# AjayGaneshC/medical-segmentation-pytorch

Measured on AMD Instinct MI355X. Metric: images/sec (whole node) + val Dice, DUCKNet-17 352x352 at 1/2/4/8 MI355X, higher is better.
Workload: dtype bf16; 1 GPU; model=DUCKNet-17, global_batch=320, per_gpu_batch=320, seq_len=123904, step=SegTrainer.train_step, image_size=352, parallelism=dp1, impl=fused, optimizer=adam, loss=ce, syncbn=False, hipgraph=True

## Files before the change

### csrc/bindings.cpp

```cpp
#include <torch/extension.h>
#include <c10/hip/HIPStream.h>

#include <algorithm>
#include <vector>

#include "launchers.h"

namespace {

hipStream_t cur_stream() { return c10::hip::getCurrentHIPStream().stream(); }

#define CHECK_DEV(t) TORCH_CHECK((t).is_cuda() && (t).is_contiguous(), #t " must be a contiguous GPU tensor")
#define CHECK_BF16(t) CHECK_DEV(t); TORCH_CHECK((t).scalar_type() == at::kBFloat16, #t " must be bf16")
#define CHECK_F32(t) CHECK_DEV(t); TORCH_CHECK((t).scalar_type() == at::kFloat, #t " must be fp32")
#define CHECK_I64(t) CHECK_DEV(t); TORCH_CHECK((t).scalar_type() == at::kLong, #t " must be int64")

inline uint16_t* bf(const at::Tensor& t) { return reinterpret_cast<uint16_t*>(t.data_ptr()); }
inline float* f32(const at::Tensor& t) { return t.data_ptr<float>(); }
inline const float* f32_opt(const c10::optional<at::Tensor>& t) {
  if (!t.has_value() || !t->defined()) return nullptr;
  CHECK_F32(*t);
  return t->data_ptr<float>();
}
inline float* f32_opt_mut(const c10::optional<at::Tensor>& t) { return const_cast<float*>(f32_opt(t)); }
// ... 1585 lines not shown
  a.Kp = (int)Kp_d;
  a.dxo = bf(dxo);
  if (bn_y.has_value() && bn_y->defined()) {
    CHECK_BF16(*bn_y); TORCH_CHECK(bn_y->numel() == nx, "bn_y numel");
    TORCH_CHECK(bn_coef.has_value() && stat_part.has_value(), "BN epilogue needs bn_coef and stat_part");
    CHECK_F32(*bn_coef); CHECK_F32(*stat_part);
    TORCH_CHECK(bn_coef->numel() >= 3 * g.Cgi && stat_part->numel() == nblk * 2 * g.Cgi, "BN epilogue shapes");
    a.bn_y = bf(*bn_y); a.bn_coef = bn_coef->data_ptr<float>(); a.stat_part = stat_part->data_ptr<float>();
  }
  a.bn_relu = bn_relu ? 1 : 0;
  a.dw = f32(dw);
  a.accum = accumulate ? 1 : 0;
  const int rc = conv_bwd_fused(a, g, cur_stream());
  TORCH_CHECK(rc == 0, "conv_bwd_fused: launch failed (", rc, ")");
}

}

extern "C" const char* msp_sources_sha();

PYBIND11_MODULE(_C, m) {
  m.doc() = "MI355X (gfx950) HIP kernels for medical_segmentation_pytorch_amd";
  m.def("conv_fwd", &conv_fwd, py::arg("xs"), py::arg("wp"), py::arg("ys"), py::arg("bias"), py::arg("stat_part"),
        py::arg("dims"), py::arg("dy"), py::arg("dx"), py::arg("trans"), py::arg("xc") = OptTensors{},
        py::arg("xrelu") = 0, py::arg("accumulate") = false, py::arg("gy") = OptTensors{},
        py::arg("gs") = OptTensors{}, py::arg("gk") = OptTensors{}, py::arg("grelu") = 0);
  m.def("conv_fwd_bn", &conv_fwd_bn, py::arg("xs"), py::arg("wp"), py::arg("ys"), py::arg("stat_part"), py::arg("dims"),
        py::arg("dy"), py::arg("dx"), py::arg("bn_y"), py::arg("bn_coef"), py::arg("relu"), py::arg("gy") = OptTensors{},
        py::arg("gs") = OptTensors{}, py::arg("gk") = OptTensors{}, py::arg("grelu") = 0);
  m.def("conv_wgrad", &conv_wgrad_t, py::arg("dys"), py::arg("xs"), py::arg("dw"), py::arg("dims"), py::arg("dy"),
        py::arg("dx"), py::arg("trans"), py::arg("xc") = OptTensors{}, py::arg("xrelu") = 0,
        py::arg("gy") = OptTensors{}, py::arg("gs") = OptTensors{}, py::arg("gk") = OptTensors{}, py::arg("grelu") = 0);
  m.def("conv_wgrad_uses_halo", &conv_wgrad_uses_halo_t);
  m.def("conv_pick_mi", &conv_pick_mi);
  m.def("conv_rows_alloc", &conv_rows_alloc);
  m.def("conv_stat_blocks", &conv_stat_blocks_t, py::arg("dims"), py::arg("dy"), py::arg("dx"), py::arg("trans") = false,
        py::arg("bwd") = false, py::arg("bne") = false);
  m.def("conv_uses_halo", &conv_uses_halo_t, py::arg("dims"), py::arg("dy"), py::arg("dx"), py::arg("trans"),
        py::arg("bwd") = false);
  m.def("conv_set_halo", [](bool on) { conv_set_halo(on ? 1 : 0); });
  m.def("conv_set_halo_split", [](int64_t mode) { conv_set_halo_split((int)mode); });
  m.def("conv_set_gemm", [](bool on) { conv_gemm_set(on ? 1 : 0); });
  m.def("conv_gemm_force_cfg", [](int64_t c) { conv_gemm_force_cfg((int)c); });
  m.def("conv_gemm_num_cfgs", []() { return conv_gemm_num_cfgs(); });
  m.def("conv_gemm_stamp_buffer", [](c10::optional<at::Tensor> buf) {
    if (!buf.has_value()) return conv_gemm_stamp_buffer(nullptr, 0);
    TORCH_CHECK(buf->is_cuda() && buf->is_contiguous() && buf->scalar_type() == at::kLong && buf->dim() == 2 &&
                    buf->size(1) == 4, "conv_gemm_stamp_buffer: a contiguous int64 [blocks][4] device tensor");
    return conv_gemm_stamp_buffer(buf->data_ptr(), buf->size(0));
  });
  m.def("conv_set_wgrad_gemm", [](int64_t mode) { conv_wgrad_gemm_set((int)mode); });
  m.def("conv_wgrad_gemm_force_cfg", [](int64_t c) { conv_wgrad_gemm_force_cfg((int)c); });
  m.def("conv_wgrad_gemm_num_cfgs", []() { return conv_wgrad_gemm_num_cfgs(); });
  m.def("conv_uses_wgrad_gemm", [](std::vector<int64_t> dims, std::vector<int64_t> dy, std::vector<int64_t> dx, bool trans) {
    return conv_wgrad_gemm_ok(make_geom(dims, dy, dx), trans);
  });
  m.def("conv_uses_gemm", [](std::vector<int64_t> dims, std::vector<int64_t> dy, std::vector<int64_t> dx, bool trans) {
    return conv_gemm_ok(make_geom(dims, dy, dx), trans);
  });
  m.def("conv_set_phase", [](bool on) { conv_set_phase(on ? 1 : 0); });
  m.def("pack_weight", &pack_weight_t);
  m.def("unpack_wgrad", &unpack_wgrad_t, py::arg("src"), py::arg("dst"), py::arg("nrow"), py::arg("nch"),
        py::arg("T"), py::arg("Cpk"), py::arg("Ktot"), py::arg("t_base"), py::arg("c_base"), py::arg("s_row"),
        py::arg("s_ch"), py::arg("accumulate"), py::arg("nrep") = 1, py::arg("rep_stride") = 0);
  m.def("conv_wgrad_replicas", &conv_wgrad_replicas_t, py::arg("dims"), py::arg("dy"), py::arg("dx"), py::arg("trans"),
        py::arg("bwd") = false, py::arg("pro") = false);
  m.def("pack_batch", &pack_batch_t);
  m.def("pack_per_block", &pack_per_block);
  m.def("bn_partial_blocks", [](int64_t P, int64_t Cp) { return bn_partial_blocks(P, Cp); });
  m.def("sum_stats", &sum_stats_t, py::arg("inputs"), py::arg("out"), py::arg("part"), py::arg("P"), py::arg("Cp"),
        py::arg("coefs") = OptTensors{}, py::arg("relu_mask") = 0);
  m.def("bn_reduce_partials", &bn_reduce_partials_t);
  m.def("bn_reduce_splits", [](int64_t nblk) { return bn_reduce_splits(nblk); });
  m.def("bn_collapse", &bn_collapse_t);
  m.def("bn_finalize", &bn_finalize_t);
  m.def("bn_reduce_finalize", &bn_reduce_finalize_t);
  m.def("bn_reduce_bwd_finalize", &bn_reduce_bwd_finalize_t);
  m.def("bn_rf_chunks", [](int64_t Cp) { return bn_rf_chunks((int)Cp); });
  m.def("bn_act_apply", &bn_act_apply_t);
  m.def("bn_act_apply_relu6", &bn_act_apply_relu6_t);
  m.def("bn_add_act", &bn_add_act_t);
  m.def("gconv_fwd", &gconv_fwd_t);
  m.def("relu6", &relu6_t);
  m.def("relu6_bwd", &relu6_bwd_t);
  m.def("bn_aug_mask", &bn_aug_mask_t);
  m.def("gconv_dgrad", &gconv_dgrad_t);
  m.def("gconv_wgrad_slices", &gconv_wgrad_slices_t);
  m.def("gconv_wgrad", &gconv_wgrad_t);
  m.def("gconv_mfma", &gconv_mfma_t);
  m.def("gconv_wgrad_mfma", &gconv_wgrad_mfma_t);
  m.def("gconv_wgrad_mfma_slices", &gconv_wgrad_mfma_slices_t);
  m.def("aug_gray_scratch_doubles", &aug_gray_scratch_doubles);
  m.def("bn_act_bwd_partial", &bn_act_bwd_partial_t);
  m.def("bn_bwd_finalize", &bn_bwd_finalize_t, py::arg("tmp"), py::arg("C"), py::arg("Cp"), py::arg("count"),
        py::arg("stats"), py::arg("dgamma"), py::arg("dbeta"), py::arg("coef"), py::arg("pscale") = 1.0);
  m.def("bn_act_bwd_apply", &bn_act_bwd_apply_t);
  m.def("bn_act_bwd_apply_part", &bn_act_bwd_apply_part_t);
  m.def("bn_tail_partial", &bn_tail_partial_t);
  m.def("bn_tail_apply", &bn_tail_apply_t, py::arg("dz"), py::arg("ys"), py::arg("ostats"), py::arg("ocoef"),
        py::arg("orelu"), py::arg("y"), py::arg("st"), py::arg("coef"), py::arg("relu_mask"), py::arg("dy"),
        py::arg("P"), py::arg("Cp"), py::arg("g") = py::none());
  m.def("bn_tail_blocks", [](int64_t P, int64_t Cp) { return bn_tail_blocks(P, (int)Cp); });
  m.attr("kTailMax") = kTailMax;
  m.attr("kTailMaxCp") = kTailMaxCp;
  m.def("nchw_to_nhwc", &nchw_to_nhwc_t);
  m.def("nhwc_to_nchw", &nhwc_to_nchw_t);
// ... 135 lines not shown
```

### csrc/conv_wgrad_gemm.hip

```cpp
#include <algorithm>

#include "common.h"
#include "launchers.h"

namespace {

typedef float f32x16_t __attribute__((ext_vector_type(16)));
typedef short s16x4_t __attribute__((ext_vector_type(4)));
typedef __attribute__((address_space(3))) uint8_t lds_u8_t;

DEVI f32x16_t mfma32(const uint4& a, const uint4& b, f32x16_t c) {
#ifdef GK_KO_MFMA
  c[0] += __uint_as_float(a.x ^ b.y);
  return c;
#else
  return __builtin_amdgcn_mfma_f32_32x32x16_bf16(as_bf16x8(a), as_bf16x8(b), c, 0, 0, 0);
#endif
}

__device__ __attribute__((aligned(64))) uint4 g_wg_zero_page[4];

DEVI void glds16(const void* src, uint32_t lds) {
#ifdef GK_KO_DMA
  return;
#endif
  unsigned keep;
  asm volatile("s_mov_b32 %0, m0\n\ts_mov_b32 m0, %2\n\ts_nop 0\n\tglobal_load_lds_dwordx4 %1, off\n\ts_mov_b32 m0, %0"
               : "=&s"(keep) : "v"(src), "s"(lds) : "memory");
}

DEVI uint2 tr_read(const uint8_t* p) {
#ifdef GK_KO_LDS
  return make_uint2((uint32_t)(uintptr_t)p, 1u);
#endif
  s16x4_t v = __builtin_amdgcn_ds_read_tr16_b64_v4i16((s16x4_t __attribute__((address_space(3)))*)(p));
  union { s16x4_t s; uint2 u; } c; c.s = v; return c.u;
}

struct FastDiv { uint32_t mul, shr; };
DEVI uint32_t fdiv_u(uint32_t n, FastDiv f) {
  return (uint32_t)(((uint64_t)__umulhi(n, f.mul) + n) >> f.shr);
}
FastDiv make_fastdiv(uint32_t d) {
  FastDiv f{0, 0};
  if (d <= 1) return f;
  uint32_t l = 0;
  while ((1ull << l) < d) ++l;
  f.mul = (uint32_t)((((1ull << l) - d) << 32) / d + 1);
  f.shr = l;
  return f;
}

constexpr int kBP = 64;

template <int R>
DEVI int chunk_swz(int row) { return R == 64 ? 0 : (R == 128 ? ((row >> 1) & 1) : (row & 3)); }

struct WgGeom {
  long M;
  int KT, n_co, n_k, stages_per_split, nstages;
  FastDiv d_ohw, d_ow;
  int kw, ty0, tys, tx0, txs;
};

template <int WM, int WN, int FM, int FN, bool PRO>
__global__ __launch_bounds__(64 * WM * WN, 2) void conv_wgrad_gemm_kernel(WgradPtrs P, float* __restrict__ dw,
                                                                          ConvGeom g, WgGeom wg) {
  constexpr int NW = WM * WN, NT = 64 * NW;
  constexpr int TCO = 32 * WM * FM, TK = 32 * WN * FN;
  constexpr int RA = TCO * 2, RB = TK * 2;
  constexpr int A_BYTES = kBP * RA, B_BYTES = kBP * RB, STAGE = A_BYTES + B_BYTES;
  constexpr int A_RPI = 1024 / RA, B_RPI = 1024 / RB;
  constexpr int A_INS = kBP / A_RPI / NW, B_INS = kBP / B_RPI / NW;
  static_assert((RA == 64 || RA == 128 || RA % 256 == 0) && (RB == 64 || RB == 128 || RB % 256 == 0), "row bytes");
  static_assert(RA <= 1024 && RB <= 1024 && A_INS * A_RPI * NW == kBP && B_INS * B_RPI * NW == kBP, "DMA split");
  static_assert(!PRO || B_RPI % 4 == 0, "prologue: one channel vector per lane (B rows <= 256 B)");
  extern __shared__ __attribute__((aligned(16))) uint8_t smem[];

  const int tid = threadIdx.x, lane = tid & 63, wave = __builtin_amdgcn_readfirstlane(tid >> 6);
  const uint32_t sbase = (uint32_t)(uintptr_t)(lds_u8_t*)smem;

  const int nwg = gridDim.x, orig = blockIdx.x;
  const int xq = nwg / 8, xr = nwg % 8, xcd = orig % 8;
  const int wgid = (xcd < xr ? xcd * (xq + 1) : xr * (xq + 1) + (xcd - xr) * xq) + orig / 8;
  const int ntile = wg.n_co * wg.n_k;
  const int split = wgid / ntile, tile = wgid - split * ntile;
  const int co_t = tile % wg.n_co, k_t = tile / wg.n_co;
  const int co0 = co_t * TCO, k0 = k_t * TK;
  const int rows = g.Go * g.Cgo, Cip = g.Gi * g.Cgi;
  const int st0 = split * wg.stages_per_split;
  const int nst = max(0, min(wg.stages_per_split, wg.nstages - st0));
  const uint16_t* zero = reinterpret_cast<const uint16_t*>(g_wg_zero_page);

  const uint16_t* a_base[A_INS];
  int a_row[A_INS];
#pragma unroll
  for (int j = 0; j < A_INS; ++j) {
    const int row = (j * NW + wave) * A_RPI + (lane * 16) / RA;
    const int slot = ((lane * 16) % RA) / 16;
    const int col = 32 * ((slot >> 2) ^ chunk_swz<RA>(row)) + 8 * (slot & 3);
    const int co = co0 + col;
    a_row[j] = row;
    if (co < rows) {
      const int og = co / g.Cgo;
      a_base[j] = P.dy[og] + (co - og * g.Cgo);
    } else {
      a_base[j] = nullptr;
    }
  }
  const uint16_t* b_base[B_INS];
  int b_row[B_INS], b_dy[B_INS], b_dx[B_INS];
  int b_ci = 0, b_gi = 0;
#pragma unroll
  for (int j = 0; j < B_INS; ++j) {
    const int row = (j * NW + wave) * B_RPI + (lane * 16) / RB;
    const int slot = ((lane * 16) % RB) / 16;
    const int col = 32 * ((slot >> 2) ^ chunk_swz<RB>(row)) + 8 * (slot & 3);
    const int k = k0 + col;
    b_row[j] = row;
    if (k < wg.KT) {
      const int t = k / Cip, rem = k - (k / Cip) * Cip;
      const int gi = rem / g.Cgi, ci = rem - gi * g.Cgi;
      const int tr = t / wg.kw, tc = t - (t / wg.kw) * wg.kw;
      b_dy[j] = wg.ty0 + tr * wg.tys;
      b_dx[j] = wg.tx0 + tc * wg.txs;
      const uint16_t* xg = P.x[0];
#pragma unroll
      for (int q = 1; q < kMaxGroups; ++q) xg = gi == q ? P.x[q] : xg;
      b_base[j] = xg + ci;
      b_ci = ci; b_gi = gi;
    } else {
      b_base[j] = nullptr; b_dy[j] = 0; b_dx[j] = 0;
    }
  }
  float psc[8], psh[8];
  bool prelu = false, pro_on = false;
  if constexpr (PRO) {
    const float* cf = P.xc[0];
#pragma unroll
    for (int q = 1; q < kMaxGroups; ++q) cf = b_gi == q ? P.xc[q] : cf;
    pro_on = cf != nullptr && b_base[0] != nullptr;
    prelu = (P.xrelu >> b_gi) & 1u;
#pragma unroll
    for (int e = 0; e < 8; ++e) { psc[e] = 1.f; psh[e] = 0.f; }
    if (pro_on) { load8f(cf + b_ci, psc); load8f(cf + g.Cgi + b_ci, psh); }
  }

  auto stage = [&](int s, uint32_t sb) -> unsigned {
    const long mb = (long)(st0 + s) * kBP;
#pragma unroll
    for (int j = 0; j < A_INS; ++j) {
      const long m = mb + a_row[j];
      const void* src = (a_base[j] != nullptr && m < wg.M) ? (const void*)(a_base[j] + m * g.Cgo) : (const void*)zero;
      glds16(src, sb + (j * NW + wave) * 1024);
    }
    unsigned ok = 0;
#pragma unroll
    for (int j = 0; j < B_INS; ++j) {
      const long m = mb + b_row[j];
      const void* src = zero;
      if (b_base[j] != nullptr && m < wg.M) {
        const uint32_t mu = (uint32_t)m;
        const uint32_t n = fdiv_u(mu, wg.d_ohw);
        const uint32_t r = mu - n * (uint32_t)(g.OH * g.OW);
        const uint32_t oh = fdiv_u(r, wg.d_ow);
        const int ow = (int)(r - oh * (uint32_t)g.OW);
        const int ih = (int)oh * g.stride + b_dy[j], iw = ow * g.stride + b_dx[j];
        if ((unsigned)ih < (unsigned)g.IH && (unsigned)iw < (unsigned)g.IW) {
          src = b_base[j] + ((long)((int)n * g.IH + ih) * g.IW + iw) * g.Cgi;
          ok |= 1u << j;
        }
      }
      glds16(src, sb + A_BYTES + (j * NW + wave) * 1024);
    }
    return ok;
  };

  const int wm = wave / WN, wn = wave - (wave / WN) * WN;
  const int gq = lane >> 4, li = lane & 15, lq = li >> 2, lp = li & 3;
  auto tr_addr = [&](int R, int row, int col) -> int {
    const int sw = R == 64 ? 0 : (R == 128 ? ((row >> 1) & 1) : (row & 3));
    return row * R + (((col >> 5) ^ sw) << 6) + ((col & 31) << 1);
  };
  int a_off[FM][2], b_off[FN][2];
#pragma unroll
  for (int i = 0; i < FM; ++i)
#pragma unroll
    for (int hh = 0; hh < 2; ++hh)
      a_off[i][hh] = tr_addr(RA, 8 * (gq >> 1) + 4 * hh + lq, wm * FM * 32 + i * 32 + 16 * (gq & 1) + 4 * lp);
#pragma unroll
  for (int j = 0; j < FN; ++j)
#pragma unroll
    for (int hh = 0; hh < 2; ++hh)
      b_off[j][hh] = A_BYTES + tr_addr(RB, 8 * (gq >> 1) + 4 * hh + lq, wn * FN * 32 + j * 32 + 16 * (gq & 1) + 4 * lp);

  f32x16_t acc[FM][FN];
#pragma unroll
  for (int i = 0; i < FM; ++i)
#pragma unroll
    for (int j = 0; j < FN; ++j)
#pragma unroll
      for (int e = 0; e < 16; ++e) acc[i][j][e] = 0.f;

  unsigned ok_cur = 0, ok_nxt = 0;
  if (nst > 0) ok_cur = stage(0, sbase);
  for (int s = 0; s < nst; ++s) {
    asm volatile("s_waitcnt vmcnt(0)" ::: "memory");
    const uint32_t cur = (s & 1) * STAGE;
    if constexpr (PRO) {
      if (pro_on) {
#pragma unroll
        for (int j = 0; j < B_INS; ++j) {
          if (!((ok_cur >> j) & 1u)) continue;
          uint4* v = reinterpret_cast<uint4*>(smem + cur + A_BYTES + (j * NW + wave) * 1024 + lane * 16);
          *v = affine8(*v, psc, psh, prelu);
        }
      }
      asm volatile("s_waitcnt lgkmcnt(0)" ::: "memory");
    }
    __builtin_amdgcn_s_barrier();
    __builtin_amdgcn_sched_barrier(0);
    if (s + 1 < nst) ok_nxt = stage(s + 1, sbase + ((s + 1) & 1) * STAGE);
    const uint8_t* sp = smem + cur;
#pragma unroll
    for (int ks = 0; ks < kBP / 16; ++ks) {
      uint4 af[FM], bf[FN];
#pragma unroll
      for (int i = 0; i < FM; ++i) {
        const uint2 lo = tr_read(sp + a_off[i][0] + ks * 16 * RA);
        const uint2 hi = tr_read(sp + a_off[i][1] + ks * 16 * RA);
        af[i] = make_uint4(lo.x, lo.y, hi.x, hi.y);
      }
#pragma unroll
      for (int j = 0; j < FN; ++j) {
        const uint2 lo = tr_read(sp + b_off[j][0] + ks * 16 * RB);
        const uint2 hi = tr_read(sp + b_off[j][1] + ks * 16 * RB);
        bf[j] = make_uint4(lo.x, lo.y, hi.x, hi.y);
      }
#pragma unroll
      for (int i = 0; i < FM; ++i)
#pragma unroll
        for (int j = 0; j < FN; ++j) acc[i][j] = mfma32(af[i], bf[j], acc[i][j]);
    }
    ok_cur = ok_nxt;
  }

  float* slab = dw + (long)split * rows * wg.KT;
  const int kc = k0 + wn * FN * 32 + (lane & 31);
  const int lh = lane >> 5;
#pragma unroll
  for (int j = 0; j < FN; ++j) {
    const int k = kc + 32 * j;
    if (k >= wg.KT) continue;
#pragma unroll
    for (int i = 0; i < FM; ++i)
#pragma unroll
      for (int e = 0; e < 16; ++e) {
        const int co = co0 + wm * FM * 32 + i * 32 + 8 * (e >> 2) + 4 * lh + (e & 3);
        if (co < rows) slab[(long)co * wg.KT + k] = acc[i][j][e];
      }
  }
}

constexpr bool wg_pro_ok(int wn, int fn) { return 32 * wn * fn <= 128; }

struct WgCfg { int wm, wn, fm, fn; };
constexpr WgCfg kWgCfgs[] = {
    {2, 2, 2, 2},
    {1, 4, 1, 1},
    {2, 2, 1, 2},
    {2, 2, 2, 1},
    {1, 4, 2, 1},
    {2, 2, 4, 1},
    {2, 4, 4, 2},
    {2, 4, 2, 2},
    {4, 2, 2, 2},
};
constexpr int kNumWgCfgs = sizeof(kWgCfgs) / sizeof(kWgCfgs[0]);

int g_wg_mode = -1;
int g_wg_cfg = -1;
constexpr long g_wg_blocks = 512;
constexpr double g_wg_stage_cost = 96.0;

void wg_env() {
  if (g_wg_mode < 0) {
    const char* e = getenv("MSP_WGRAD_GEMM");
    g_wg_mode = e == nullptr ? 1 : (e[0] == '0' ? 0 : (e[0] == '2' ? 2 : 1));
  }
}

int wg_pick(int rows, int KT, bool pro) {
  if (g_wg_cfg >= 0 && (!pro || wg_pro_ok(kWgCfgs[g_wg_cfg].wn, kWgCfgs[g_wg_cfg].fn))) return g_wg_cfg;
  int best = 0;
  double best_cost = 1e30;
  for (int c = 0; c < kNumWgCfgs; ++c) {
    if (pro && !wg_pro_ok(kWgCfgs[c].wn, kWgCfgs[c].fn)) continue;
    const int tco = 32 * kWgCfgs[c].wm * kWgCfgs[c].fm, tk = 32 * kWgCfgs[c].wn * kWgCfgs[c].fn;
    const double nt = (double)cdiv(rows, tco) * cdiv(KT, tk);
    const double cost = nt * ((double)tco * tk + g_wg_stage_cost * (tco + tk));
    if (cost < best_cost) { best_cost = cost; best = c; }
  }
  return best;
}

bool wg_tap_grid(const ConvGeom& g, WgGeom& w) {
  for (int kw = 1; kw <= g.T; ++kw) {
    if (g.T % kw != 0) continue;
    const int kh = g.T / kw;
    w.kw = kw; w.ty0 = g.dy[0]; w.tx0 = g.dx[0];
    w.tys = kh > 1 ? g.dy[kw] - g.dy[0] : 0;
    w.txs = kw > 1 ? g.dx[1] - g.dx[0] : 0;
    bool ok = true;
    for (int t = 0; t < g.T && ok; ++t) ok = g.dy[t] == w.ty0 + (t / kw) * w.tys && g.dx[t] == w.tx0 + (t % kw) * w.txs;
    if (ok) return true;
  }
  return false;
}

struct WgPlan { int cfg; WgGeom w; long blocks; int nsplit; };

WgPlan wg_plan(const ConvGeom& g, bool pro) {
  WgPlan p{};
  p.cfg = wg_pick(g.Go * g.Cgo, g.T * g.Gi * g.Cgi, pro);
  const WgCfg& c = kWgCfgs[p.cfg];
  WgGeom& w = p.w;
  (void)wg_tap_grid(g, w);
  w.M = (long)g.N * g.OH * g.OW;
  w.KT = g.T * g.Gi * g.Cgi;
  w.n_co = cdiv(g.Go * g.Cgo, 32 * c.wm * c.fm);
  w.n_k = cdiv(w.KT, 32 * c.wn * c.fn);
  w.nstages = (int)((w.M + kBP - 1) / kBP);
  const long ntile = (long)w.n_co * w.n_k;
  const long target = c.wm * c.wn >= 8 ? g_wg_blocks / 2 : g_wg_blocks;
  long ns = std::max(1L, std::min((long)w.nstages, target / std::max(1L, ntile)));
  w.stages_per_split = (int)((w.nstages + ns - 1) / ns);
  ns = (w.nstages + w.stages_per_split - 1) / w.stages_per_split;
  p.nsplit = (int)ns;
  p.blocks = ns * ntile;
  w.d_ohw = make_fastdiv((uint32_t)(g.OH * g.OW));
  w.d_ow = make_fastdiv((uint32_t)g.OW);
  return p;
}

template <int WM, int WN, int FM, int FN>
int launch_wg(const WgradPtrs& P, float* dw, const ConvGeom& g, const WgPlan& p, bool pro, hipStream_t s) {
  constexpr int LDS = 2 * kBP * (32 * WM * FM + 32 * WN * FN) * 2;
  static bool attr[2] = {false, false};
  if (pro) {
    if constexpr (!wg_pro_ok(WN, FN)) {
      return 1;
    } else {
    if (!attr[1]) {
      (void)hipFuncSetAttribute(reinterpret_cast<const void*>(&conv_wgrad_gemm_kernel<WM, WN, FM, FN, true>),
                                hipFuncAttributeMaxDynamicSharedMemorySize, LDS);
      attr[1] = true;
    }
    hipLaunchKernelGGL((conv_wgrad_gemm_kernel<WM, WN, FM, FN, true>), dim3((unsigned)p.blocks), dim3(64 * WM * WN),
                       LDS, s, P, dw, g, p.w);
    return 0;
    }
  }
  if (!attr[0]) {
    (void)hipFuncSetAttribute(reinterpret_cast<const void*>(&conv_wgrad_gemm_kernel<WM, WN, FM, FN, false>),
                              hipFuncAttributeMaxDynamicSharedMemorySize, LDS);
    attr[0] = true;
  }
  hipLaunchKernelGGL((conv_wgrad_gemm_kernel<WM, WN, FM, FN, false>), dim3((unsigned)p.blocks), dim3(64 * WM * WN), LDS,
                     s, P, dw, g, p.w);
  return 0;
}


}

bool conv_wgrad_gemm_ok(const ConvGeom& g, bool trans) {
  wg_env();
  if (!g_wg_mode || trans || g.Cgi % 8 != 0 || g.Cgo % 8 != 0) return false;
  WgGeom w{};
  if (!wg_tap_grid(g, w)) return false;
  const long M = (long)g.N * g.OH * g.OW;
  return M < (1L << 31) - 2 * kBP;
}

int conv_wgrad_gemm_replicas(const ConvGeom& g, bool pro) {
  wg_env();
  return wg_plan(g, pro).nsplit;
}

void conv_wgrad_gemm_set(int mode) { wg_env(); g_wg_mode = mode < 0 ? 0 : (mode > 2 ? 2 : mode); }
int conv_wgrad_gemm_mode() { wg_env(); return g_wg_mode; }
void conv_wgrad_gemm_force_cfg(int cfg) { wg_env(); g_wg_cfg = (cfg >= 0 && cfg < kNumWgCfgs) ? cfg : -1; }
int conv_wgrad_gemm_num_cfgs() { return kNumWgCfgs; }

int conv_wgrad_gemm(const WgradPtrs& P, float* dw, const ConvGeom& g, bool prologue, hipStream_t s) {
  const WgPlan p = wg_plan(g, prologue);
  switch (p.cfg) {
    case 0: return launch_wg<2, 2, 2, 2>(P, dw, g, p, prologue, s);
    case 1: return launch_wg<1, 4, 1, 1>(P, dw, g, p, prologue, s);
    case 2: return launch_wg<2, 2, 1, 2>(P, dw, g, p, prologue, s);
    case 3: return launch_wg<2, 2, 2, 1>(P, dw, g, p, prologue, s);
    case 4: return launch_wg<1, 4, 2, 1>(P, dw, g, p, prologue, s);
    case 5: return launch_wg<2, 2, 4, 1>(P, dw, g, p, prologue, s);
    case 6: return launch_wg<2, 4, 4, 2>(P, dw, g, p, prologue, s);
    case 7: return launch_wg<2, 4, 2, 2>(P, dw, g, p, prologue, s);
    case 8: return launch_wg<4, 2, 2, 2>(P, dw, g, p, prologue, s);
  }
  return 1;
}
```

### csrc/launchers.h

```cpp
#pragma once
#include <hip/hip_runtime.h>
#include <stdint.h>

constexpr int kMaxTaps = 49;

constexpr int kMaxGroups = 8;
struct ConvGeom {
  int N, IH, IW;
  int Gi, Cgi;
  int OH, OW;
  int Go, Cgo, Cgo_l;
  int T, Kp;
  int stride;
  int dy[kMaxTaps], dx[kMaxTaps];
};

struct ConvArgs {
  const uint16_t* x[kMaxGroups];
  uint16_t* y[kMaxGroups];
  const uint16_t* w;
  const float* bias;
  float* stat_part;
  const uint16_t* bn_y;
  const float* bn_coef;
  int bn_relu;
  const float* xc[kMaxGroups];
  unsigned xrelu;
  int accum;
  const uint16_t* gy[kMaxGroups];
  const float* gs[kMaxGroups];
  const float* gk[kMaxGroups];
  unsigned grelu;
  ConvGeom g;
};

struct WgradPtrs {
  const uint16_t* dy[kMaxGroups];
  const uint16_t* x[kMaxGroups];
  const float* xc[kMaxGroups];
  unsigned xrelu;
  const uint16_t* gy[kMaxGroups];
  const float* gs[kMaxGroups];
  const float* gk[kMaxGroups];
  unsigned grelu;
};

bool conv_wgrad_gemm_ok(const ConvGeom& g, bool trans);
int conv_wgrad_gemm_replicas(const ConvGeom& g, bool pro = false);
int conv_wgrad_gemm(const WgradPtrs& P, float* dw, const ConvGeom& g, bool prologue, hipStream_t s);
void conv_wgrad_gemm_set(int mode);
int conv_wgrad_gemm_mode();
void conv_wgrad_gemm_force_cfg(int cfg);
int conv_wgrad_gemm_num_cfgs();

int conv_pick_mi(int rows);
int conv_rows_alloc(int rows);
void conv_set_halo(int on);
void conv_set_halo_split(int mode);
void conv_set_phase(int on);
bool conv_uses_halo(const ConvGeom& g, bool trans, bool bwd = false);
long conv_stat_blocks(const ConvGeom& g, bool trans = false, bool bwd = false, bool bne = false);
bool conv_wgrad_uses_halo(const ConvGeom& g, bool trans);
int conv_igemm(const ConvArgs& a, bool trans, hipStream_t s);
const char* conv_error_string(int rc);

bool conv_gemm_ok(const ConvGeom& g, bool trans);
long conv_gemm_stat_blocks(const ConvGeom& g);
int conv_gemm(const ConvArgs& a, hipStream_t s);
int conv_gemm_phase(const ConvArgs& a, const int* tA, int KW, int s_, int py, int px, int OHf, int OWf,
                    hipStream_t s);
void conv_gemm_set(int on);
void conv_gemm_force_cfg(int cfg);
int conv_gemm_num_cfgs();
int conv_gemm_stamp_buffer(void* buf, long cap);
int conv_plan_selfcheck(int verbose);
int conv_wgrad_replicas(const ConvGeom& g, bool trans, bool bwd = false, bool pro = false);
int conv_wgrad(const uint16_t* const* dy, const uint16_t* const* x, float* dw, const ConvGeom& g, bool trans,
               const float* const* xc, unsigned xrelu, hipStream_t s, const uint16_t* const* gy = nullptr,
               const float* const* gs = nullptr, const float* const* gk = nullptr, unsigned grelu = 0);
void pack_weight(const float* src, uint16_t* dst, int nrow, int nch, int T, int Cpk, int Kp, int t_base,
                 int c_base, long s_row, long s_ch, hipStream_t s);
void pack_batch(const int64_t* jobs, const int* prefix, int njobs, int total_blocks, hipStream_t s);
int pack_per_block();
void unpack_wgrad(const float* src, float* dst, int nrow, int nch, int T, int Cpk, int Ktot, int t_base, int c_base,
                  long s_row, long s_ch, bool accumulate, int nrep, long rep_stride, hipStream_t s);

constexpr int kMaxSumInputs = 8;
constexpr int kTailMax = 6;
constexpr int kTailMaxCp = 512;
long bn_partial_blocks(long P, int Cp);
long bn_tail_blocks(long P, int Cp);
void bn_tail_partial(const uint16_t* dz, const uint16_t* ys, const float* ostats, const float* ocoef, int orelu, int k,
                     const uint16_t* const* y, const float* const* st, unsigned relu, float* part, long P, int Cp,
                     hipStream_t s);
void bn_tail_apply(const uint16_t* dz, const uint16_t* ys, const float* ostats, const float* ocoef, int orelu, int k,
                   const uint16_t* const* y, const float* const* st, const float* const* coef, unsigned relu,
                   uint16_t* const* dy, long P, int Cp, hipStream_t s, uint16_t* g = nullptr);
void sum_stats(const uint16_t* const* inputs, const float* const* coefs, unsigned relu_mask, int k, uint16_t* out,
               float* part, long P, int Cp, hipStream_t s);
int bn_reduce_splits(long nblk);
void bn_reduce_partials(const float* part, long nblk, int width, int col_off, int Cp, double* tmp, hipStream_t s);
void bn_collapse(const double* tmp, int S, int Cp, double* out, hipStream_t s);
void bn_finalize(const double* tmp, int S, int C, int Cp, float count, const float* gamma, const float* beta,
                 float* running_mean, float* running_var, float momentum, float eps, int training,
                 float* scale, float* shift, float* mean, float* invstd, hipStream_t s);
int bn_rf_chunks(int Cp);
// ... 283 lines not shown
```

Before: 687.9 images/sec.

## Add multi-stage LDS ring pipeline and incremental addressing to wgrad GEMM

Turns the weight-gradient GEMM's fixed double buffer into a configurable NS-stage ring with a BP-pixel stage depth. Global-to-LDS DMA issues are interleaved across the k-slices of the MFMA loop, and vmcnt waits are partial instead of full drains. Per-stage pixel-to-(n,oh,ow) divisions are replaced by incremental carry-based pointer advances, and an m0 save/restore is dropped. The 96K-LDS configs now default to a 3-stage ring, which uses more LDS per block and may lower occupancy. Split-count override and timestamp instrumentation hooks are also added.

New measurement: 687.8 images/sec. No clear change (-0.0%).

```diff
diff --git a/csrc/bindings.cpp b/csrc/bindings.cpp
--- a/csrc/bindings.cpp
+++ b/csrc/bindings.cpp
@@ -1661,6 +1661,24 @@
   m.def("conv_set_wgrad_gemm", [](int64_t mode) { conv_wgrad_gemm_set((int)mode); });
   m.def("conv_wgrad_gemm_force_cfg", [](int64_t c) { conv_wgrad_gemm_force_cfg((int)c); });
   m.def("conv_wgrad_gemm_num_cfgs", []() { return conv_wgrad_gemm_num_cfgs(); });
+  m.def("conv_wgrad_gemm_force_splits", [](int64_t n) { conv_wgrad_gemm_force_splits((int)n); });
+  m.def("conv_wgrad_gemm_ring", [](int64_t c) {
+    int ns = 0, bp = 0;
+    bool pro = false;
+    TORCH_CHECK(conv_wgrad_gemm_ring((int)c, &ns, &bp, &pro), "conv_wgrad_gemm_ring: no configuration ", c);
+    return std::make_tuple(ns, bp, pro);
+  });
+  m.def("conv_wgrad_gemm_forced", []() {
+    int cfg = -1, ns = -1;
+    conv_wgrad_gemm_forced(&cfg, &ns);
+    return std::make_pair(cfg, ns);
+  });
+  m.def("conv_wgrad_gemm_stamp_buffer", [](c10::optional<at::Tensor> buf) {
+    if (!buf.has_value()) return conv_wgrad_gemm_stamp_buffer(nullptr, 0);
+    TORCH_CHECK(buf->is_cuda() && buf->is_contiguous() && buf->scalar_type() == at::kLong && buf->dim() == 2 &&
+                    buf->size(1) == 6, "conv_wgrad_gemm_stamp_buffer: a contiguous int64 [blocks][6] device tensor");
+    return conv_wgrad_gemm_stamp_buffer(buf->data_ptr(), buf->size(0));
+  });
   m.def("conv_uses_wgrad_gemm", [](std::vector<int64_t> dims, std::vector<int64_t> dy, std::vector<int64_t> dx, bool trans) {
     return conv_wgrad_gemm_ok(make_geom(dims, dy, dx), trans);
   });
diff --git a/csrc/conv_wgrad_gemm.hip b/csrc/conv_wgrad_gemm.hip
--- a/csrc/conv_wgrad_gemm.hip
+++ b/csrc/conv_wgrad_gemm.hip
@@ -1,4 +1,5 @@
 #include <algorithm>
+#include <type_traits>
 
 #include "common.h"
 #include "launchers.h"
@@ -20,13 +21,27 @@
 
 __device__ __attribute__((aligned(64))) uint4 g_wg_zero_page[4];
 
+#ifdef GK_STAMP
+DEVI unsigned long long wg_clock() {
+  unsigned long long t;
+  __builtin_amdgcn_sched_barrier(0);
+  asm volatile("s_memrealtime %0\n\ts_waitcnt lgkmcnt(0)" : "=s"(t)::"memory");
+  __builtin_amdgcn_sched_barrier(0);
+  return t;
+}
+#endif
+
 DEVI void glds16(const void* src, uint32_t lds) {
 #ifdef GK_KO_DMA
   return;
 #endif
-  unsigned keep;
-  asm volatile("s_mov_b32 %0, m0\n\ts_mov_b32 m0, %2\n\ts_nop 0\n\tglobal_load_lds_dwordx4 %1, off\n\ts_mov_b32 m0, %0"
-               : "=&s"(keep) : "v"(src), "s"(lds) : "memory");
+  asm volatile("s_mov_b32 m0, %1\n\ts_nop 0\n\tglobal_load_lds_dwordx4 %0, off" ::"v"(src), "s"(lds) : "memory");
+}
+
+template <int N>
+DEVI void wait_vm() {
+  static_assert(N >= 0 && N < 64, "vmcnt is a 6-bit count");
+  asm volatile("s_waitcnt vmcnt(%0)" ::"n"(N) : "memory");
 }
 
 DEVI uint2 tr_read(const uint8_t* p) {
@@ -51,7 +66,7 @@
   return f;
 }
 
-constexpr int kBP = 64;
+constexpr int kSplitPx = 64;
 
 template <int R>
 DEVI int chunk_swz(int row) { return R == 64 ? 0 : (R == 128 ? ((row >> 1) & 1) : (row & 3)); }
@@ -61,21 +76,35 @@
   int KT, n_co, n_k, stages_per_split, nstages;
   FastDiv d_ohw, d_ow;
   int kw, ty0, tys, tx0, txs;
+  int q_n, q_oh, q_ow;
+  long img_bytes, img_step0, img_step1;
+#ifdef GK_STAMP
+  unsigned long long* stamp;
+  long stamp_cap;
+#endif
 };
 
-template <int WM, int WN, int FM, int FN, bool PRO>
+template <int WM, int WN, int FM, int FN, bool PRO, int NS, int BP>
 __global__ __launch_bounds__(64 * WM * WN, 2) void conv_wgrad_gemm_kernel(WgradPtrs P, float* __restrict__ dw,
                                                                           ConvGeom g, WgGeom wg) {
   constexpr int NW = WM * WN, NT = 64 * NW;
   constexpr int TCO = 32 * WM * FM, TK = 32 * WN * FN;
   constexpr int RA = TCO * 2, RB = TK * 2;
-  constexpr int A_BYTES = kBP * RA, B_BYTES = kBP * RB, STAGE = A_BYTES + B_BYTES;
+  constexpr int A_BYTES = BP * RA, B_BYTES = BP * RB, STAGE = A_BYTES + B_BYTES;
   constexpr int A_RPI = 1024 / RA, B_RPI = 1024 / RB;
-  constexpr int A_INS = kBP / A_RPI / NW, B_INS = kBP / B_RPI / NW;
+  constexpr int A_INS = BP / A_RPI / NW, B_INS = BP / B_RPI / NW;
+  constexpr int NI = A_INS + B_INS;
+  constexpr int KS = BP / 16;
+  static_assert(NS >= 2 && NS <= 5 && BP % 16 == 0 && kSplitPx % BP == 0, "ring");
   static_assert((RA == 64 || RA == 128 || RA % 256 == 0) && (RB == 64 || RB == 128 || RB % 256 == 0), "row bytes");
-  static_assert(RA <= 1024 && RB <= 1024 && A_INS * A_RPI * NW == kBP && B_INS * B_RPI * NW == kBP, "DMA split");
+  static_assert(RA <= 1024 && RB <= 1024 && A_INS * A_RPI * NW == BP && B_INS * B_RPI * NW == BP, "DMA split");
   static_assert(!PRO || B_RPI % 4 == 0, "prologue: one channel vector per lane (B rows <= 256 B)");
+  static_assert((NS - 1) * B_INS <= 32, "in-image masks of the stages in flight: one 32-bit queue");
   extern __shared__ __attribute__((aligned(16))) uint8_t smem[];
+#ifdef GK_STAMP
+  const unsigned long long ts0 = wg_clock();
+  unsigned long long ts1 = ts0, tsb = 0, bsum = 0;
+#endif
 
   const int tid = threadIdx.x, lane = tid & 63, wave = __builtin_amdgcn_readfirstlane(tid >> 6);
   const uint32_t sbase = (uint32_t)(uintptr_t)(lds_u8_t*)smem;
@@ -88,11 +117,13 @@
   const int co_t = tile % wg.n_co, k_t = tile / wg.n_co;
   const int co0 = co_t * TCO, k0 = k_t * TK;
   const int rows = g.Go * g.Cgo, Cip = g.Gi * g.Cgi;
-  const int st0 = split * wg.stages_per_split;
-  const int nst = max(0, min(wg.stages_per_split, wg.nstages - st0));
-  const uint16_t* zero = reinterpret_cast<const uint16_t*>(g_wg_zero_page);
-
-  const uint16_t* a_base[A_INS];
+  const long px0 = (long)split * wg.stages_per_split * kSplitPx;
+  const long px1 = min(wg.M, px0 + (long)wg.stages_per_split * kSplitPx);
+  const int nst = px1 > px0 ? (int)((px1 - px0 + BP - 1) / BP) : 0;
+  const uint8_t* zero = reinterpret_cast<const uint8_t*>(g_wg_zero_page);
+  asm volatile("" : "+s"(zero));
+
+  const uint8_t* a_ptr[A_INS];
   int a_row[A_INS];
 #pragma unroll
   for (int j = 0; j < A_INS; ++j) {
@@ -100,80 +131,87 @@
     const int slot = ((lane * 16) % RA) / 16;
     const int col = 32 * ((slot >> 2) ^ chunk_swz<RA>(row)) + 8 * (slot & 3);
     const int co = co0 + col;
-    a_row[j] = row;
     if (co < rows) {
       const int og = co / g.Cgo;
-      a_base[j] = P.dy[og] + (co - og * g.Cgo);
+      a_ptr[j] = reinterpret_cast<const uint8_t*>(P.dy[og] + (co - og * g.Cgo) + (px0 + row) * g.Cgo);
+      a_row[j] = row;
     } else {
-      a_base[j] = nullptr;
-    }
-  }
-  const uint16_t* b_base[B_INS];
-  int b_row[B_INS], b_dy[B_INS], b_dx[B_INS];
+      a_ptr[j] = zero;
+      a_row[j] = 1 << 30;
+    }
+  }
+  const int a_step = BP * g.Cgo * 2;
+  int rem = (int)min(wg.M - px0, (long)(1 << 29));
+  const uint8_t* b_img[B_INS];
+  int b_n[B_INS], b_oh[B_INS], b_ow[B_INS], b_dy[B_INS], b_dx[B_INS];
   int b_ci = 0, b_gi = 0;
+  bool b_k0 = false;
 #pragma unroll
   for (int j = 0; j < B_INS; ++j) {
     const int row = (j * NW + wave) * B_RPI + (lane * 16) / RB;
     const int slot = ((lane * 16) % RB) / 16;
     const int col = 32 * ((slot >> 2) ^ chunk_swz<RB>(row)) + 8 * (slot & 3);
     const int k = k0 + col;
-    b_row[j] = row;
+    const uint32_t mu = (uint32_t)(px0 + row);
+    const uint32_t n = fdiv_u(mu, wg.d_ohw);
+    const uint32_t r = mu - n * (uint32_t)(g.OH * g.OW);
+    const uint32_t oh = fdiv_u(r, wg.d_ow);
+    b_n[j] = (int)n; b_oh[j] = (int)oh; b_ow[j] = (int)(r - oh * (uint32_t)g.OW);
     if (k < wg.KT) {
-      const int t = k / Cip, rem = k - (k / Cip) * Cip;
-      const int gi = rem / g.Cgi, ci = rem - gi * g.Cgi;
+      const int t = k / Cip, rm = k - (k / Cip) * Cip;
+      const int gi = rm / g.Cgi, ci = rm - gi * g.Cgi;
       const int tr = t / wg.kw, tc = t - (t / wg.kw) * wg.kw;
       b_dy[j] = wg.ty0 + tr * wg.tys;
       b_dx[j] = wg.tx0 + tc * wg.txs;
       const uint16_t* xg = P.x[0];
 #pragma unroll
       for (int q = 1; q < kMaxGroups; ++q) xg = gi == q ? P.x[q] : xg;
-      b_base[j] = xg + ci;
+      b_img[j] = reinterpret_cast<const uint8_t*>(xg + ci) + (long)n * wg.img_bytes;
       b_ci = ci; b_gi = gi;
+      if (j == 0) b_k0 = true;
     } else {
-      b_base[j] = nullptr; b_dy[j] = 0; b_dx[j] = 0;
-    }
-  }
+      b_img[j] = zero; b_dy[j] = -(1 << 22); b_dx[j] = 0;
+    }
+  }
+  const int cgi2 = g.Cgi * 2;
   float psc[8], psh[8];
   bool prelu = false, pro_on = false;
   if constexpr (PRO) {
     const float* cf = P.xc[0];
 #pragma unroll
     for (int q = 1; q < kMaxGroups; ++q) cf = b_gi == q ? P.xc[q] : cf;
-    pro_on = cf != nullptr && b_base[0] != nullptr;
+    pro_on = cf != nullptr && b_k0;
     prelu = (P.xrelu >> b_gi) & 1u;
 #pragma unroll
     for (int e = 0; e < 8; ++e) { psc[e] = 1.f; psh[e] = 0.f; }
     if (pro_on) { load8f(cf + b_ci, psc); load8f(cf + g.Cgi + b_ci, psh); }
   }
 
-  auto stage = [&](int s, uint32_t sb) -> unsigned {
-    const long mb = (long)(st0 + s) * kBP;
-#pragma unroll
-    for (int j = 0; j < A_INS; ++j) {
-      const long m = mb + a_row[j];
-      const void* src = (a_base[j] != nullptr && m < wg.M) ? (const void*)(a_base[j] + m * g.Cgo) : (const void*)zero;
+  auto issue = [&](int i, uint32_t sb, unsigned& ok) {
+    if (i < A_INS) {
+      const int j = i;
+      const void* src = a_row[j] < rem ? (const void*)a_ptr[j] : (const void*)zero;
       glds16(src, sb + (j * NW + wave) * 1024);
-    }
-    unsigned ok = 0;
-#pragma unroll
-    for (int j = 0; j < B_INS; ++j) {
-      const long m = mb + b_row[j];
-      const void* src = zero;
-      if (b_base[j] != nullptr && m < wg.M) {
-        const uint32_t mu = (uint32_t)m;
-        const uint32_t n = fdiv_u(mu, wg.d_ohw);
-        const uint32_t r = mu - n * (uint32_t)(g.OH * g.OW);
-        const uint32_t oh = fdiv_u(r, wg.d_ow);
-        const int ow = (int)(r - oh * (uint32_t)g.OW);
-        const int ih = (int)oh * g.stride + b_dy[j], iw = ow * g.stride + b_dx[j];
-        if ((unsigned)ih < (unsigned)g.IH && (unsigned)iw < (unsigned)g.IW) {
-          src = b_base[j] + ((long)((int)n * g.IH + ih) * g.IW + iw) * g.Cgi;
-          ok |= 1u << j;
-        }
-      }
+      a_ptr[j] += a_step;
+    } else {
+      const int j = i - A_INS;
+      const int ih = __mul24(b_oh[j], g.stride) + b_dy[j], iw = __mul24(b_ow[j], g.stride) + b_dx[j];
+      const bool in = (b_n[j] < g.N) & ((unsigned)ih < (unsigned)g.IH) & ((unsigned)iw < (unsigned)g.IW);
+      const uint32_t off = __umul24(__umul24((unsigned)ih, (unsigned)g.IW) + (unsigned)iw, (unsigned)cgi2);
+      const uint8_t* at = b_img[j] + off;
+      asm volatile("" : "+v"(at));
+      const void* src = in ? (const void*)at : (const void*)zero;
       glds16(src, sb + A_BYTES + (j * NW + wave) * 1024);
-    }
-    return ok;
+      ok |= in ? (1u << j) : 0u;
+      int ow = b_ow[j] + wg.q_ow;
+      const bool c1 = ow >= g.OW;
+      b_ow[j] = c1 ? ow - g.OW : ow;
+      int oh = b_oh[j] + wg.q_oh + (c1 ? 1 : 0);
+      const bool c2 = oh >= g.OH;
+      b_oh[j] = c2 ? oh - g.OH : oh;
+      b_n[j] += wg.q_n + (c2 ? 1 : 0);
+      b_img[j] += c2 ? wg.img_step1 : wg.img_step0;
+    }
   };
 
   const int wm = wave / WN, wn = wave - (wave / WN) * WN;
@@ -202,28 +240,51 @@
 #pragma unroll
       for (int e = 0; e < 16; ++e) acc[i][j][e] = 0.f;
 
-  unsigned ok_cur = 0, ok_nxt = 0;
-  if (nst > 0) ok_cur = stage(0, sbase);
-  for (int s = 0; s < nst; ++s) {
-    asm volatile("s_waitcnt vmcnt(0)" ::: "memory");
-    const uint32_t cur = (s & 1) * STAGE;
+  int cb = 0, ib = 0;
+  unsigned okq = 0;
+#pragma unroll
+  for (int p = 0; p < NS - 1; ++p) {
+    if (p < nst) {
+      unsigned ok = 0;
+#pragma unroll
+      for (int i = 0; i < NI; ++i) issue(i, sbase + ib * STAGE, ok);
+      okq |= ok << (p * B_INS);
+      rem -= BP;
+      ++ib;
+    }
+  }
+  if (ib == NS) ib = 0;
+
+  auto iter = [&](auto infl, const bool more, const bool first) {
+    constexpr int INFL = decltype(infl)::value;
+    wait_vm<INFL * NI>();
+    const uint32_t cur = cb * STAGE;
     if constexpr (PRO) {
       if (pro_on) {
 #pragma unroll
         for (int j = 0; j < B_INS; ++j) {
-          if (!((ok_cur >> j) & 1u)) continue;
+          if (!((okq >> j) & 1u)) continue;
           uint4* v = reinterpret_cast<uint4*>(smem + cur + A_BYTES + (j * NW + wave) * 1024 + lane * 16);
           *v = affine8(*v, psc, psh, prelu);
         }
       }
-      asm volatile("s_waitcnt lgkmcnt(0)" ::: "memory");
-    }
+    }
+    asm volatile("s_waitcnt lgkmcnt(0)" ::: "memory");
     __builtin_amdgcn_s_barrier();
     __builtin_amdgcn_sched_barrier(0);
-    if (s + 1 < nst) ok_nxt = stage(s + 1, sbase + ((s + 1) & 1) * STAGE);
+#ifdef GK_STAMP
+    tsb = wg_clock();
+#endif
+    const uint32_t nxt = sbase + ib * STAGE;
+    unsigned ok = 0;
     const uint8_t* sp = smem + cur;
 #pragma unroll
-    for (int ks = 0; ks < kBP / 16; ++ks) {
+    for (int ks = 0; ks < KS; ++ks) {
+      if (more) {
+#pragma unroll
+        for (int i = 0; i < NI; ++i)
+          if ((i * KS) / NI == ks) issue(i, nxt, ok);
+      }
       uint4 af[FM], bf[FN];
 #pragma unroll
       for (int i = 0; i < FM; ++i) {
@@ -237,13 +298,41 @@
         const uint2 hi = tr_read(sp + b_off[j][1] + ks * 16 * RB);
         bf[j] = make_uint4(lo.x, lo.y, hi.x, hi.y);
       }
+#ifdef GK_STAMP
+      if (ks == 0) {
+        const unsigned long long t = wg_clock();
+        bsum += t - tsb;
+        if (first) ts1 = t;
+      }
+#endif
 #pragma unroll
       for (int i = 0; i < FM; ++i)
 #pragma unroll
         for (int j = 0; j < FN; ++j) acc[i][j] = mfma32(af[i], bf[j], acc[i][j]);
     }
-    ok_cur = ok_nxt;
-  }
+    okq >>= B_INS;
+    cb = cb + 1 == NS ? 0 : cb + 1;
+    if (more) {
+      okq |= ok << ((NS - 2) * B_INS);
+      rem -= BP;
+      ib = ib + 1 == NS ? 0 : ib + 1;
+    }
+  };
+
+  int s = 0;
+  for (; s + (NS - 2) < nst; ++s) iter(std::integral_constant<int, NS - 2>{}, s + NS - 1 < nst, s == 0);
+  if constexpr (NS >= 5) {
+    if (nst - 1 - s == 2) { iter(std::integral_constant<int, 2>{}, false, s == 0); ++s; }
+  }
+  if constexpr (NS >= 4) {
+    if (nst - 1 - s == 1) { iter(std::integral_constant<int, 1>{}, false, s == 0); ++s; }
+  }
+  if constexpr (NS >= 3) {
+    if (nst - 1 - s == 0) { iter(std::integral_constant<int, 0>{}, false, s == 0); ++s; }
+  }
+#ifdef GK_STAMP
+  const unsigned long long ts2 = wg_clock();
+#endif
 
   float* slab = dw + (long)split * rows * wg.KT;
   const int kc = k0 + wn * FN * 32 + (lane & 31);
@@ -260,26 +349,51 @@
         if (co < rows) slab[(long)co * wg.KT + k] = acc[i][j][e];
       }
   }
+#ifdef GK_STAMP
+  const unsigned long long ts3 = wg_clock();
+  if (tid == 0 && wg.stamp != nullptr && wgid < wg.stamp_cap) {
+    unsigned long long* sp = wg.stamp + 6 * (long)wgid;
+    sp[0] = ts0; sp[1] = ts1; sp[2] = ts2; sp[3] = ts3; sp[4] = bsum; sp[5] = (unsigned long long)nst;
+  }
+#endif
 }
 
 constexpr bool wg_pro_ok(int wn, int fn) { return 32 * wn * fn <= 128; }
 
-struct WgCfg { int wm, wn, fm, fn; };
+#ifndef WG_NS_256
+#define WG_NS_256 2
+#endif
+#ifndef WG_BP_256
+#define WG_BP_256 64
+#endif
+#ifndef WG_NS_96K
+#define WG_NS_96K 3
+#endif
+#ifndef WG_BP_96K
+#define WG_BP_96K 64
+#endif
+
+struct WgCfg { int wm, wn, fm, fn, ns, bp; };
 constexpr WgCfg kWgCfgs[] = {
-    {2, 2, 2, 2},
-    {1, 4, 1, 1},
-    {2, 2, 1, 2},
-    {2, 2, 2, 1},
-    {1, 4, 2, 1},
-    {2, 2, 4, 1},
-    {2, 4, 4, 2},
-    {2, 4, 2, 2},
-    {4, 2, 2, 2},
+    {2, 2, 2, 2, 2, 64},
+    {1, 4, 1, 1, 2, 64},
+    {2, 2, 1, 2, 2, 64},
+    {2, 2, 2, 1, 2, 64},
+    {1, 4, 2, 1, 2, 64},
+    {2, 2, 4, 1, 2, 64},
+    {2, 4, 4, 2, WG_NS_256, WG_BP_256},
+    {2, 4, 2, 2, WG_NS_96K, WG_BP_96K},
+    {4, 2, 2, 2, WG_NS_96K, WG_BP_96K},
 };
 constexpr int kNumWgCfgs = sizeof(kWgCfgs) / sizeof(kWgCfgs[0]);
 
 int g_wg_mode = -1;
 int g_wg_cfg = -1;
+int g_wg_splits = -1;
+#ifdef GK_STAMP
+unsigned long long* g_wg_stamp = nullptr;
+long g_wg_stamp_cap = 0;
+#endif
 constexpr long g_wg_blocks = 512;
 constexpr double g_wg_stage_cost = 96.0;
 
@@ -330,47 +444,64 @@
   w.KT = g.T * g.Gi * g.Cgi;
   w.n_co = cdiv(g.Go * g.Cgo, 32 * c.wm * c.fm);
   w.n_k = cdiv(w.KT, 32 * c.wn * c.fn);
-  w.nstages = (int)((w.M + kBP - 1) / kBP);
+  w.nstages = (int)((w.M + kSplitPx - 1) / kSplitPx);
   const long ntile = (long)w.n_co * w.n_k;
   const long target = c.wm * c.wn >= 8 ? g_wg_blocks / 2 : g_wg_blocks;
   long ns = std::max(1L, std::min((long)w.nstages, target / std::max(1L, ntile)));
+  if (g_wg_splits > 0) ns = std::min((long)w.nstages, (long)g_wg_splits);
   w.stages_per_split = (int)((w.nstages + ns - 1) / ns);
   ns = (w.nstages + w.stages_per_split - 1) / w.stages_per_split;
   p.nsplit = (int)ns;
   p.blocks = ns * ntile;
   w.d_ohw = make_fastdiv((uint32_t)(g.OH * g.OW));
   w.d_ow = make_fastdiv((uint32_t)g.OW);
+  const int ohw = g.OH * g.OW;
+  w.q_n = c.bp / ohw;
+  w.q_oh = (c.bp - w.q_n * ohw) / g.OW;
+  w.q_ow = c.bp - w.q_n * ohw - w.q_oh * g.OW;
+  w.img_bytes = (long)g.IH * g.IW * g.Cgi * 2;
+  w.img_step0 = w.q_n * w.img_bytes;
+  w.img_step1 = (w.q_n + 1) * w.img_bytes;
+#ifdef GK_STAMP
+  w.stamp = g_wg_stamp; w.stamp_cap = g_wg_stamp_cap;
+#endif
   return p;
 }
 
-template <int WM, int WN, int FM, int FN>
+template <int WM, int WN, int FM, int FN, int NS, int BP>
 int launch_wg(const WgradPtrs& P, float* dw, const ConvGeom& g, const WgPlan& p, bool pro, hipStream_t s) {
-  constexpr int LDS = 2 * kBP * (32 * WM * FM + 32 * WN * FN) * 2;
+  constexpr int LDS = NS * BP * (32 * WM * FM + 32 * WN * FN) * 2;
+  static_assert(LDS <= 160 * 1024, "LDS budget");
   static bool attr[2] = {false, false};
   if (pro) {
     if constexpr (!wg_pro_ok(WN, FN)) {
       return 1;
     } else {
     if (!attr[1]) {
-      (void)hipFuncSetAttribute(reinterpret_cast<const void*>(&conv_wgrad_gemm_kernel<WM, WN, FM, FN, true>),
+      (void)hipFuncSetAttribute(reinterpret_cast<const void*>(&conv_wgrad_gemm_kernel<WM, WN, FM, FN, true, NS, BP>),
                                 hipFuncAttributeMaxDynamicSharedMemorySize, LDS);
       attr[1] = true;
     }
-    hipLaunchKernelGGL((conv_wgrad_gemm_kernel<WM, WN, FM, FN, true>), dim3((unsigned)p.blocks), dim3(64 * WM * WN),
-                       LDS, s, P, dw, g, p.w);
+    hipLaunchKernelGGL((conv_wgrad_gemm_kernel<WM, WN, FM, FN, true, NS, BP>), dim3((unsigned)p.blocks),
+                       dim3(64 * WM * WN), LDS, s, P, dw, g, p.w);
     return 0;
     }
   }
   if (!attr[0]) {
-    (void)hipFuncSetAttribute(reinterpret_cast<const void*>(&conv_wgrad_gemm_kernel<WM, WN, FM, FN, false>),
+    (void)hipFuncSetAttribute(reinterpret_cast<const void*>(&conv_wgrad_gemm_kernel<WM, WN, FM, FN, false, NS, BP>),
                               hipFuncAttributeMaxDynamicSharedMemorySize, LDS);
     attr[0] = true;
   }
-  hipLaunchKernelGGL((conv_wgrad_gemm_kernel<WM, WN, FM, FN, false>), dim3((unsigned)p.blocks), dim3(64 * WM * WN), LDS,
-                     s, P, dw, g, p.w);
+  hipLaunchKernelGGL((conv_wgrad_gemm_kernel<WM, WN, FM, FN, false, NS, BP>), dim3((unsigned)p.blocks),
+                     dim3(64 * WM * WN), LDS, s, P, dw, g, p.w);
   return 0;
 }
 
+template <int I>
+int launch_cfg(const WgradPtrs& P, float* dw, const ConvGeom& g, const WgPlan& p, bool pro, hipStream_t s) {
+  constexpr WgCfg c = kWgCfgs[I];
+  return launch_wg<c.wm, c.wn, c.fm, c.fn, c.ns, c.bp>(P, dw, g, p, pro, s);
+}
 
 }
 
@@ -379,8 +510,11 @@
   if (!g_wg_mode || trans || g.Cgi % 8 != 0 || g.Cgo % 8 != 0) return false;
   WgGeom w{};
   if (!wg_tap_grid(g, w)) return false;
+  if ((long)g.IH * g.IW >= (1L << 24) || (long)g.IH * g.IW * g.Cgi * 2 >= (1L << 31) || g.Cgi * 2 >= (1 << 24) ||
+      (long)g.OH * g.stride >= (1L << 22) || (long)g.OW * g.stride >= (1L << 22))
+    return false;
   const long M = (long)g.N * g.OH * g.OW;
-  return M < (1L << 31) - 2 * kBP;
+  return M < (1L << 31) - 2 * kSplitPx;
 }
 
 int conv_wgrad_gemm_replicas(const ConvGeom& g, bool pro) {
@@ -391,20 +525,39 @@
 void conv_wgrad_gemm_set(int mode) { wg_env(); g_wg_mode = mode < 0 ? 0 : (mode > 2 ? 2 : mode); }
 int conv_wgrad_gemm_mode() { wg_env(); return g_wg_mode; }
 void conv_wgrad_gemm_force_cfg(int cfg) { wg_env(); g_wg_cfg = (cfg >= 0 && cfg < kNumWgCfgs) ? cfg : -1; }
+void conv_wgrad_gemm_force_splits(int nsplit) { wg_env(); g_wg_splits = nsplit > 0 ? nsplit : -1; }
 int conv_wgrad_gemm_num_cfgs() { return kNumWgCfgs; }
+void conv_wgrad_gemm_forced(int* cfg, int* nsplit) { *cfg = g_wg_cfg; *nsplit = g_wg_splits; }
+bool conv_wgrad_gemm_ring(int cfg, int* ns, int* bp, bool* pro) {
+  if (cfg < 0 || cfg >= kNumWgCfgs) return false;
+  *ns = kWgCfgs[cfg].ns; *bp = kWgCfgs[cfg].bp;
+  *pro = wg_pro_ok(kWgCfgs[cfg].wn, kWgCfgs[cfg].fn);
+  return true;
+}
+
+int conv_wgrad_gemm_stamp_buffer(void* buf, long cap) {
+#ifdef GK_STAMP
+  g_wg_stamp = static_cast<unsigned long long*>(buf);
+  g_wg_stamp_cap = buf != nullptr ? cap : 0;
+  return 1;
+#else
+  (void)buf; (void)cap;
+  return 0;
+#endif
+}
 
 int conv_wgrad_gemm(const WgradPtrs& P, float* dw, const ConvGeom& g, bool prologue, hipStream_t s) {
   const WgPlan p = wg_plan(g, prologue);
   switch (p.cfg) {
-    case 0: return launch_wg<2, 2, 2, 2>(P, dw, g, p, prologue, s);
-    case 1: return launch_wg<1, 4, 1, 1>(P, dw, g, p, prologue, s);
-    case 2: return launch_wg<2, 2, 1, 2>(P, dw, g, p, prologue, s);
-    case 3: return launch_wg<2, 2, 2, 1>(P, dw, g, p, prologue, s);
-    case 4: return launch_wg<1, 4, 2, 1>(P, dw, g, p, prologue, s);
-    case 5: return launch_wg<2, 2, 4, 1>(P, dw, g, p, prologue, s);
-    case 6: return launch_wg<2, 4, 4, 2>(P, dw, g, p, prologue, s);
-    case 7: return launch_wg<2, 4, 2, 2>(P, dw, g, p, prologue, s);
-    case 8: return launch_wg<4, 2, 2, 2>(P, dw, g, p, prologue, s);
+    case 0: return launch_cfg<0>(P, dw, g, p, prologue, s);
+    case 1: return launch_cfg<1>(P, dw, g, p, prologue, s);
+    case 2: return launch_cfg<2>(P, dw, g, p, prologue, s);
+    case 3: return launch_cfg<3>(P, dw, g, p, prologue, s);
+    case 4: return launch_cfg<4>(P, dw, g, p, prologue, s);
+    case 5: return launch_cfg<5>(P, dw, g, p, prologue, s);
+    case 6: return launch_cfg<6>(P, dw, g, p, prologue, s);
+    case 7: return launch_cfg<7>(P, dw, g, p, prologue, s);
+    case 8: return launch_cfg<8>(P, dw, g, p, prologue, s);
   }
   return 1;
 }
diff --git a/csrc/launchers.h b/csrc/launchers.h
--- a/csrc/launchers.h
+++ b/csrc/launchers.h
@@ -51,7 +51,11 @@
 void conv_wgrad_gemm_set(int mode);
 int conv_wgrad_gemm_mode();
 void conv_wgrad_gemm_force_cfg(int cfg);
+void conv_wgrad_gemm_force_splits(int nsplit);
+void conv_wgrad_gemm_forced(int* cfg, int* nsplit);
 int conv_wgrad_gemm_num_cfgs();
+bool conv_wgrad_gemm_ring(int cfg, int* ns, int* bp, bool* pro);
+int conv_wgrad_gemm_stamp_buffer(void* buf, long cap);
 
 int conv_pick_mi(int rows);
 int conv_rows_alloc(int rows);
```
